# nmonette/TO-UED

Hardware: NVIDIA B200
Metric: gridworld agent env-steps/sec incl. LPG update (higher is better)
Workload: dtype f16/bf16 operands, f32 accumulate (GRU); f32 elsewhere

## Files before the change

to_ued_b200/csrc/rollout.cu:

```cuda
#include "gridworld.cuh"
#include "../../include/toued.h"

template <int O>
__global__ void __launch_bounds__(128)
rollout_kernel(const LevelRec* __restrict__ levels, const uint32_t* __restrict__ keys,
               const float* __restrict__ actor, const uint8_t* __restrict__ forced_actions,
               int32_t* __restrict__ state, int32_t* __restrict__ obs, uint8_t* __restrict__ action,
               float* __restrict__ reward, uint8_t* __restrict__ done, float* __restrict__ ep_return,
               int n_agents, int W, int L, int D, int G2, int apb, int reset_first) {
    extern __shared__ __align__(16) unsigned char smem_raw[];
    LevelRec* lv = reinterpret_cast<LevelRec*>(smem_raw);
    __shared__ __align__(8) uint64_t bar;

    const int agent0 = blockIdx.x * apb;
    const int n_here = min(apb, n_agents - agent0);
    if (threadIdx.x == 0) { mbar_init(&bar, 1); mbar_fence_init(); }
    __syncthreads();
    if (threadIdx.x == 0) {
        const uint32_t bytes = (uint32_t)(n_here * sizeof(LevelRec));
        mbar_expect_tx(&bar, bytes);
        bulk_g2s(lv, levels + agent0, bytes, &bar);
    }
    mbar_wait(&bar, 0);

    const int la = threadIdx.x / W;
    const int w = threadIdx.x - la * W;
    const int agent = agent0 + la;
    if (la >= n_here) return;
    const LevelRec& lev = lv[la];
    const float* table = actor + (size_t)agent * D * TOUED_ACT_PAD;

    Key rng;
    {
        Key ak; ak.a = keys[2 * agent]; ak.b = keys[2 * agent + 1];
        rng = split_n(ak, (uint32_t)W, (uint32_t)w);
    }

    EnvRegs s;
    if (reset_first) {
        s = env_reset(lev);
    } else {
        const int32_t ps = state[(size_t)agent * W + w];
        s.pos = st_pos(ps); s.exists = st_exists(ps); s.time = st_time(ps);
    }
    float cum = 0.0f, valid = 1.0f;
    const size_t tok0 = (size_t)agent * L * W + w;
    const size_t ob0 = (size_t)agent * (L + 1) * W + w;
    const bool write = obs != nullptr;
    if (write) obs[ob0] = pack_obs(obs_row(s, G2), s.time);

    for (int t = 0; t < L; ++t) {
        Key k_act, k_env;
        split2(rng, rng, k_act);
        split2(rng, rng, k_env);
        const float u_act = uniform_scalar(k_act);
        const StepRand<O> rnd = env_step_rand<O>(k_env);

        int a;
        {
            float z[TOUED_NUM_ACTIONS], p[TOUED_NUM_ACTIONS];
            tab_logits<TOUED_NUM_ACTIONS, TOUED_ACT_PAD>(table, D, obs_row(s, G2), s.time, z);
            softmax_portable<TOUED_NUM_ACTIONS>(z, p);
            float c[TOUED_NUM_ACTIONS];
            c[0] = p[0];
#pragma unroll
            for (int j = 1; j < TOUED_NUM_ACTIONS; ++j) c[j] = __fadd_rn(c[j - 1], p[j]);
            const float r = __fmul_rn(c[TOUED_NUM_ACTIONS - 1], __fsub_rn(1.0f, u_act));
            a = 0;
#pragma unroll
            for (int j = 0; j < TOUED_NUM_ACTIONS; ++j) a += (c[j] < r) ? 1 : 0;
        }
        if (forced_actions) a = forced_actions[tok0 + (size_t)t * W];

        bool dn;
        const float rew = env_step_apply<O>(lev, rnd, a, s, dn);

        cum = __fadd_rn(cum, __fmul_rn(rew, valid));
        valid = __fmul_rn(valid, dn ? 0.0f : 1.0f);

        if (write) {
            const size_t k = tok0 + (size_t)t * W;
            action[k] = (uint8_t)a;
            reward[k] = rew;
            done[k] = dn ? 1 : 0;
            obs[ob0 + (size_t)(t + 1) * W] = pack_obs(obs_row(s, G2), s.time);
        }
    }
    if (state) state[(size_t)agent * W + w] = pack_state(s.pos, s.exists, s.time);
    if (ep_return) ep_return[(size_t)agent * W + w] = cum;
}

extern "C" int toued_rollout(const void* levels, const uint32_t* keys, const float* actor,
                             const uint8_t* forced_actions, int32_t* state, int32_t* obs,
                             uint8_t* action, float* reward, uint8_t* done, float* ep_return,
                             int n_agents, int n_workers, int rollout_len, int obs_dim,
                             int max_grid_size, int max_n_objs, int reset_first, void* stream) {
    TOUED_CHECK(n_agents > 0 && n_workers > 0 && rollout_len > 0, "toued_rollout: empty problem");
    TOUED_CHECK(n_workers <= 128 && (128 % n_workers) == 0,
                "toued_rollout: n_workers=%d must divide 128", n_workers);
    TOUED_CHECK(max_n_objs >= 1 && max_n_objs <= 5, "toued_rollout: max_n_objs=%d not in 1..5", max_n_objs);
    TOUED_CHECK(max_grid_size * max_grid_size <= 255, "toued_rollout: max_grid_size too large");
    TOUED_CHECK(obs_dim == max_grid_size * max_grid_size * (1 << max_n_objs) + 1,
                "toued_rollout: obs_dim=%d inconsistent with grid/objs", obs_dim);
    TOUED_CHECK(rollout_len < 65536, "toued_rollout: rollout_len too large");
    TOUED_CHECK(obs == nullptr || (action && reward && done), "toued_rollout: partial trajectory buffers");
    const int apb = 128 / n_workers;
    const int blocks = (n_agents + apb - 1) / apb;
    const size_t smem = (size_t)apb * sizeof(LevelRec);
    const int G2 = max_grid_size * max_grid_size;
    cudaStream_t st = (cudaStream_t)stream;
#define LAUNCH(OO) rollout_kernel<OO><<<blocks, 128, smem, st>>>( \
        (const LevelRec*)levels, keys, actor, forced_actions, state, obs, action, reward, done, ep_return, \
        n_agents, n_workers, rollout_len, obs_dim, G2, apb, reset_first)
    switch (max_n_objs) {
        case 1: LAUNCH(1); break;
        case 2: LAUNCH(2); break;
        case 3: LAUNCH(3); break;
        case 4: LAUNCH(4); break;
        default: LAUNCH(5); break;
    }
#undef LAUNCH
    TOUED_LAUNCH_CHECK();
    return 0;
}

template <int O>
__global__ void env_step_kernel(const LevelRec* __restrict__ levels, const uint32_t* __restrict__ keys,
                                const int32_t* __restrict__ actions, int32_t* __restrict__ state,
                                int32_t* __restrict__ obs, float* __restrict__ reward,
                                uint8_t* __restrict__ done, int n_envs, int W, int G2) {
    const int g = blockIdx.x * blockDim.x + threadIdx.x;
    if (g >= n_envs) return;
    const LevelRec lev = levels[g / W];
    Key k; k.a = keys[2 * g]; k.b = keys[2 * g + 1];
    const int32_t ps = state[g];
    EnvRegs s; s.pos = st_pos(ps); s.exists = st_exists(ps); s.time = st_time(ps);
    const StepRand<O> rnd = env_step_rand<O>(k);
    bool dn;
    const float rew = env_step_apply<O>(lev, rnd, actions[g], s, dn);
    state[g] = pack_state(s.pos, s.exists, s.time);
    obs[g] = pack_obs(obs_row(s, G2), s.time);
    reward[g] = rew;
    done[g] = dn ? 1 : 0;
}

__global__ void env_reset_kernel(const LevelRec* __restrict__ levels, int32_t* __restrict__ state,
                                 int32_t* __restrict__ obs, int n_envs, int W, int G2) {
    const int g = blockIdx.x * blockDim.x + threadIdx.x;
    if (g >= n_envs) return;
    const LevelRec lev = levels[g / W];
    const EnvRegs s = env_reset(lev);
    state[g] = pack_state(s.pos, s.exists, s.time);
    if (obs) obs[g] = pack_obs(obs_row(s, G2), s.time);
}

extern "C" int toued_env_step(const void* levels, const uint32_t* keys, const int32_t* actions,
                              int32_t* state, int32_t* obs, float* reward, uint8_t* done,
                              int n_agents, int n_workers, int max_grid_size, int max_n_objs, void* stream) {
    TOUED_CHECK(n_agents > 0 && n_workers > 0, "toued_env_step: empty problem");
    TOUED_CHECK(max_n_objs >= 1 && max_n_objs <= 5, "toued_env_step: max_n_objs=%d not in 1..5", max_n_objs);
    const int n = n_agents * n_workers, G2 = max_grid_size * max_grid_size;
    cudaStream_t st = (cudaStream_t)stream;
#define LAUNCH(OO) env_step_kernel<OO><<<(n + 127) / 128, 128, 0, st>>>((const LevelRec*)levels, keys, actions, \
        state, obs, reward, done, n, n_workers, G2)
    switch (max_n_objs) {
        case 1: LAUNCH(1); break; case 2: LAUNCH(2); break; case 3: LAUNCH(3); break;
        case 4: LAUNCH(4); break; default: LAUNCH(5); break;
    }
#undef LAUNCH
    TOUED_LAUNCH_CHECK();
    return 0;
}

extern "C" int toued_env_reset(const void* levels, int32_t* state, int32_t* obs, int n_agents,
                               int n_workers, int max_grid_size, void* stream) {
    TOUED_CHECK(n_agents > 0 && n_workers > 0, "toued_env_reset: empty problem");
    const int n = n_agents * n_workers;
    env_reset_kernel<<<(n + 127) / 128, 128, 0, (cudaStream_t)stream>>>(
        (const LevelRec*)levels, state, obs, n, n_workers, max_grid_size * max_grid_size);
    TOUED_LAUNCH_CHECK();
    return 0;
}
```

Measured before the change: 471.5 million.

## Spread each rollout env across a lane group to parallelize RNG and stores

Each environment is now handled by a group of G lanes instead of a single thread. The lanes split the per-step RNG draws and forced-action loads across a window of G steps, broadcast them with shuffles, step the env redundantly, and each lane writes one step's outputs. G is picked automatically when there are few envs (or set via an environment variable) so the grid gains threads and latency hiding. The G=1 path software-pipelines the next step's draws ahead of the current step. The cost is redundant env computation, shuffle overhead, a serial RNG split chain per window, and more template instantiations.

Result: slower. 422.7 million, median of 6 (-10.3%).

```diff
diff --git a/to_ued_b200/csrc/rollout.cu b/to_ued_b200/csrc/rollout.cu
--- a/to_ued_b200/csrc/rollout.cu
+++ b/to_ued_b200/csrc/rollout.cu
@@ -1,19 +1,29 @@
+#include <stdlib.h>
 #include "gridworld.cuh"
 #include "../../include/toued.h"
 
-template <int O>
+template <int G, typename T>
+__device__ __forceinline__ T grp_bcast(T v, int src, unsigned mask) {
+    if constexpr (G == 1) return v;
+    else return __shfl_sync(mask, v, src, G);
+}
+
+template <int O, int G>
 __global__ void __launch_bounds__(128)
 rollout_kernel(const LevelRec* __restrict__ levels, const uint32_t* __restrict__ keys,
                const float* __restrict__ actor, const uint8_t* __restrict__ forced_actions,
                int32_t* __restrict__ state, int32_t* __restrict__ obs, uint8_t* __restrict__ action,
                float* __restrict__ reward, uint8_t* __restrict__ done, float* __restrict__ ep_return,
-               int n_agents, int W, int L, int D, int G2, int apb, int reset_first) {
+               int n_agents, int W, int L, int D, int G2, int reset_first) {
     extern __shared__ __align__(16) unsigned char smem_raw[];
     LevelRec* lv = reinterpret_cast<LevelRec*>(smem_raw);
     __shared__ __align__(8) uint64_t bar;
-
-    const int agent0 = blockIdx.x * apb;
-    const int n_here = min(apb, n_agents - agent0);
+    constexpr int EPB = 128 / G;
+
+    const int e0 = blockIdx.x * EPB;
+    const int n_envs = n_agents * W;
+    const int agent0 = e0 / W;
+    const int n_here = min((e0 + EPB - 1) / W + 1, n_agents) - agent0;
     if (threadIdx.x == 0) { mbar_init(&bar, 1); mbar_fence_init(); }
     __syncthreads();
     if (threadIdx.x == 0) {
@@ -23,11 +33,13 @@
     }
     mbar_wait(&bar, 0);
 
-    const int la = threadIdx.x / W;
-    const int w = threadIdx.x - la * W;
-    const int agent = agent0 + la;
-    if (la >= n_here) return;
-    const LevelRec& lev = lv[la];
+    const int e = e0 + (int)threadIdx.x / G;
+    const int j = (int)threadIdx.x % G;
+    if (e >= n_envs) return;
+    const int agent = e / W;
+    const int w = e - agent * W;
+    const unsigned gmask = G == 32 ? 0xffffffffu : ((1u << G) - 1u) << ((threadIdx.x & 31) & ~(G - 1));
+    const LevelRec& lev = lv[agent - agent0];
     const float* table = actor + (size_t)agent * D * TOUED_ACT_PAD;
 
     Key rng;
@@ -47,47 +59,101 @@
     const size_t tok0 = (size_t)agent * L * W + w;
     const size_t ob0 = (size_t)agent * (L + 1) * W + w;
     const bool write = obs != nullptr;
-    if (write) obs[ob0] = pack_obs(obs_row(s, G2), s.time);
-
-    for (int t = 0; t < L; ++t) {
-        Key k_act, k_env;
-        split2(rng, rng, k_act);
-        split2(rng, rng, k_env);
-        const float u_act = uniform_scalar(k_act);
-        const StepRand<O> rnd = env_step_rand<O>(k_env);
-
-        int a;
-        {
-            float z[TOUED_NUM_ACTIONS], p[TOUED_NUM_ACTIONS];
-            tab_logits<TOUED_NUM_ACTIONS, TOUED_ACT_PAD>(table, D, obs_row(s, G2), s.time, z);
-            softmax_portable<TOUED_NUM_ACTIONS>(z, p);
-            float c[TOUED_NUM_ACTIONS];
-            c[0] = p[0];
+    if (write && j == 0) obs[ob0] = pack_obs(obs_row(s, G2), s.time);
+
+    struct Draws { float u; StepRand<O> rnd; int fa; };
+    auto draw_window = [&](int t0) {
+        const int nw = G == 1 ? 1 : min(G, L - t0);
+        Key k_act = rng, k_env = rng;
+        for (int i = 0; i < nw; ++i) {
+            Key ka, ke;
+            split2(rng, rng, ka);
+            split2(rng, rng, ke);
+            if (i == j) { k_act = ka; k_env = ke; }
+        }
+        Draws d;
+        d.u = uniform_scalar(k_act);
+        d.rnd = env_step_rand<O>(k_env);
+        d.fa = (forced_actions && t0 + j < L) ? forced_actions[tok0 + (size_t)(t0 + j) * W] : 0;
+        return d;
+    };
+    auto run_window = [&](int t0, const Draws& mine) {
+        const int nw = G == 1 ? 1 : min(G, L - t0);
+        int32_t ob_mine = 0;
+        int a_mine = 0;
+        float rew_mine = 0.0f;
+        bool dn_mine = false;
+        for (int i = 0; i < nw; ++i) {
+            const float u_act = grp_bcast<G>(mine.u, i, gmask);
+            StepRand<O> rnd;
+            rnd.u_term = grp_bcast<G>(mine.rnd.u_term, i, gmask);
 #pragma unroll
-            for (int j = 1; j < TOUED_NUM_ACTIONS; ++j) c[j] = __fadd_rn(c[j - 1], p[j]);
-            const float r = __fmul_rn(c[TOUED_NUM_ACTIONS - 1], __fsub_rn(1.0f, u_act));
-            a = 0;
+            for (int q = 0; q < O; ++q) rnd.u_resp[q] = grp_bcast<G>(mine.rnd.u_resp[q], i, gmask);
+
+            int a;
+            {
+                float z[TOUED_NUM_ACTIONS], p[TOUED_NUM_ACTIONS];
+                tab_logits<TOUED_NUM_ACTIONS, TOUED_ACT_PAD>(table, D, obs_row(s, G2), s.time, z);
+                softmax_portable<TOUED_NUM_ACTIONS>(z, p);
+                float c[TOUED_NUM_ACTIONS];
+                c[0] = p[0];
 #pragma unroll
-            for (int j = 0; j < TOUED_NUM_ACTIONS; ++j) a += (c[j] < r) ? 1 : 0;
-        }
-        if (forced_actions) a = forced_actions[tok0 + (size_t)t * W];
-
-        bool dn;
-        const float rew = env_step_apply<O>(lev, rnd, a, s, dn);
-
-        cum = __fadd_rn(cum, __fmul_rn(rew, valid));
-        valid = __fmul_rn(valid, dn ? 0.0f : 1.0f);
-
-        if (write) {
-            const size_t k = tok0 + (size_t)t * W;
-            action[k] = (uint8_t)a;
-            reward[k] = rew;
-            done[k] = dn ? 1 : 0;
-            obs[ob0 + (size_t)(t + 1) * W] = pack_obs(obs_row(s, G2), s.time);
-        }
-    }
-    if (state) state[(size_t)agent * W + w] = pack_state(s.pos, s.exists, s.time);
-    if (ep_return) ep_return[(size_t)agent * W + w] = cum;
+                for (int q = 1; q < TOUED_NUM_ACTIONS; ++q) c[q] = __fadd_rn(c[q - 1], p[q]);
+                const float r = __fmul_rn(c[TOUED_NUM_ACTIONS - 1], __fsub_rn(1.0f, u_act));
+                a = 0;
+#pragma unroll
+                for (int q = 0; q < TOUED_NUM_ACTIONS; ++q) a += (c[q] < r) ? 1 : 0;
+            }
+            if (forced_actions) a = grp_bcast<G>(mine.fa, i, gmask);
+
+            bool dn;
+            const float rew = env_step_apply<O>(lev, rnd, a, s, dn);
+
+            cum = __fadd_rn(cum, __fmul_rn(rew, valid));
+            valid = __fmul_rn(valid, dn ? 0.0f : 1.0f);
+
+            if (i == j) { a_mine = a; rew_mine = rew; dn_mine = dn; ob_mine = pack_obs(obs_row(s, G2), s.time); }
+        }
+        if (write && j < nw) {
+            const size_t k = tok0 + (size_t)(t0 + j) * W;
+            action[k] = (uint8_t)a_mine;
+            reward[k] = rew_mine;
+            done[k] = dn_mine ? 1 : 0;
+            obs[ob0 + (size_t)(t0 + j + 1) * W] = ob_mine;
+        }
+    };
+
+    if constexpr (G == 1) {
+        Draws cur = draw_window(0);
+        int t = 0;
+        for (; t + 1 < L; ++t) {
+            const Draws nxt = draw_window(t + 1);
+            run_window(t, cur);
+            cur = nxt;
+        }
+        run_window(t, cur);
+    } else {
+        for (int t0 = 0; t0 < L; t0 += G) run_window(t0, draw_window(t0));
+    }
+    if (j == 0) {
+        if (state) state[(size_t)agent * W + w] = pack_state(s.pos, s.exists, s.time);
+        if (ep_return) ep_return[(size_t)agent * W + w] = cum;
+    }
+}
+
+#define ROLLOUT_LANE_THREADS (1 << 17)
+static int rollout_lanes(long n_envs, int L, int* G) {
+    if (const char* ev = getenv("TOUED_ROLLOUT_LANES")) {
+        const int g = atoi(ev);
+        TOUED_CHECK(g >= 1 && g <= 32 && (g & (g - 1)) == 0,
+                    "TOUED_ROLLOUT_LANES=%s: expected 1, 2, 4, 8, 16 or 32", ev);
+        *G = g;
+        return 0;
+    }
+    int g = 1;
+    while (g < 32 && 2 * g <= L && n_envs * 2 * g <= ROLLOUT_LANE_THREADS) g *= 2;
+    *G = g;
+    return 0;
 }
 
 extern "C" int toued_rollout(const void* levels, const uint32_t* keys, const float* actor,
@@ -104,21 +170,29 @@
                 "toued_rollout: obs_dim=%d inconsistent with grid/objs", obs_dim);
     TOUED_CHECK(rollout_len < 65536, "toued_rollout: rollout_len too large");
     TOUED_CHECK(obs == nullptr || (action && reward && done), "toued_rollout: partial trajectory buffers");
-    const int apb = 128 / n_workers;
-    const int blocks = (n_agents + apb - 1) / apb;
-    const size_t smem = (size_t)apb * sizeof(LevelRec);
+    const long n_envs = (long)n_agents * n_workers;
+    TOUED_CHECK(n_envs <= (1L << 31) - 256, "toued_rollout: too many environments");
+    int G;
+    if (int rc = rollout_lanes(n_envs, rollout_len, &G)) return rc;
+    const int epb = 128 / G;
+    const int blocks = (int)((n_envs + epb - 1) / epb);
+    const size_t smem = (size_t)(epb >= n_workers ? epb / n_workers : 1) * sizeof(LevelRec);
     const int G2 = max_grid_size * max_grid_size;
     cudaStream_t st = (cudaStream_t)stream;
-#define LAUNCH(OO) rollout_kernel<OO><<<blocks, 128, smem, st>>>( \
+#define LAUNCH(OO, GG) rollout_kernel<OO, GG><<<blocks, 128, smem, st>>>( \
         (const LevelRec*)levels, keys, actor, forced_actions, state, obs, action, reward, done, ep_return, \
-        n_agents, n_workers, rollout_len, obs_dim, G2, apb, reset_first)
+        n_agents, n_workers, rollout_len, obs_dim, G2, reset_first)
+#define LAUNCH_G(OO) switch (G) { \
+        case 1: LAUNCH(OO, 1); break;   case 2: LAUNCH(OO, 2); break;   case 4: LAUNCH(OO, 4); break; \
+        case 8: LAUNCH(OO, 8); break;   case 16: LAUNCH(OO, 16); break; default: LAUNCH(OO, 32); break; }
     switch (max_n_objs) {
-        case 1: LAUNCH(1); break;
-        case 2: LAUNCH(2); break;
-        case 3: LAUNCH(3); break;
-        case 4: LAUNCH(4); break;
-        default: LAUNCH(5); break;
-    }
+        case 1: LAUNCH_G(1); break;
+        case 2: LAUNCH_G(2); break;
+        case 3: LAUNCH_G(3); break;
+        case 4: LAUNCH_G(4); break;
+        default: LAUNCH_G(5); break;
+    }
+#undef LAUNCH_G
 #undef LAUNCH
     TOUED_LAUNCH_CHECK();
     return 0;
```
